# josh-holder/marl_sap

Measured on AMD Instinct MI355X. Metric: env steps/sec (whole node), 64-agent assignment env, 1/2/4/8 MI355X, higher is better.
Workload: dtype f32

## Files before the change

include/asg.h:

```cpp
#ifndef ASG_H
#define ASG_H

#include <stdint.h>

#ifdef __cplusplus
extern "C" {
#endif

#define ASG_ABI_VERSION 1

#define ASG_OK 0
#define ASG_E_INVALID_ARG (-1)
#define ASG_E_HIP (-2)
#define ASG_E_STATE (-3)
#define ASG_E_LSA_INVALID (-4)
#define ASG_E_LSA_INFEASIBLE (-5)
#define ASG_E_ACTION_RANGE (-6)

enum asg_dtype {
    ASG_F32 = 0,
    ASG_F64 = 1,
    ASG_I64 = 2,
    ASG_I32 = 3,
    ASG_BOOL = 4,
// ... 162 lines not shown
                          uint64_t seed, uint64_t counter, int64_t env_index_base, int64_t *out,
                          int32_t *status, void *hip_stream);

int asg_rollout(asg_handle *h, const asg_batch_view *b, int ts, int steps, int select_first, int select_last,
                const void *packed, const float *b1, const float *b_r0, const float *b_r1, const float *b2, int K,
                int hidden, int use_rnn, const float *h_in, int64_t h_stride, float *h_out, double epsilon,
                uint64_t seed, uint64_t counter, int32_t *status, void *hip_stream);
int asg_reset_rollout(asg_handle *h, const asg_batch_view *b, int ts, int steps, int select_last, const void *packed,
                      const float *b1, const float *b_r0, const float *b_r1, const float *b2, int K, int hidden,
                      int use_rnn, const float *h_in, int64_t h_stride, float *h_out, double epsilon, uint64_t seed,
                      uint64_t counter, int32_t *status, void *hip_stream);
int asg_step_select(asg_handle *h, const asg_batch_view *b, int ts, const void *packed, const float *b1,
                    const float *b_ih, const float *b_hh, const float *b2, int K, int hidden, const float *h_in,
                    int64_t h_stride, float *h_out, double epsilon, uint64_t seed, uint64_t counter,
                    int32_t *status, void *hip_stream);
int asg_step_forward(asg_handle *h, const asg_batch_view *b, int ts, const void *packed, const float *b1,
                     const float *b_r0, const float *b_r1, const float *b2, int K, int hidden, int use_rnn,
                     const float *h_in, int64_t h_stride, float *h_out, float *q_out, void *hip_stream);
int asg_step_forward_ex(asg_handle *h, const asg_batch_view *b, int ts, const void *packed, const float *b1,
                        const float *b_r0, const float *b_r1, const float *b2, int K, int hidden, int use_rnn,
                        const float *h_in, int64_t h_stride, float *h_out, float *q_out, int flags,
                        void *hip_stream);
int asg_reset_forward(asg_handle *h, const asg_batch_view *b, int ts, const void *packed, const float *b1,
                      const float *b_r0, const float *b_r1, const float *b2, int K, int hidden, int use_rnn,
                      const float *h_in, int64_t h_stride, float *h_out, float *q_out, void *hip_stream);
int asg_bids_select(asg_handle *h, const float *q, const int64_t q_strides[3], float *bids_out,
                    const int64_t out_strides[3], int row_softmax, int col_softmax, double noise_std, uint64_t seed,
                    uint64_t counter, void *hip_stream);
int asg_bids_select_count(asg_handle *h, const float *q, const int64_t q_strides[3], float *bids_out,
                          const int64_t out_strides[3], int row_softmax, int col_softmax, double noise_std,
                          uint64_t seed, uint64_t counter, int32_t *path_steps_out, void *hip_stream);
int asg_rollout_l2_slices(int n, int m, int L, int use_rnn);
int asg_step_select_l2_slices(int n, int m, int L);

typedef struct asg_real_handle asg_real_handle;

enum asg_real_variant { ASG_REAL_PLAIN = 0, ASG_REAL_POWER = 1, ASG_REAL_INTERFERENCE = 2 };

typedef struct {
    int64_t num_envs;
    int32_t n, m, T, L;
    int32_t N, M;
    double lambda_;
    const double *T_trans;
    const double *task_prios;
    int32_t variant;
    int32_t bids_as_actions;
    uint64_t seed;
    int64_t env_index_base;
    const int32_t *sat_freq_bands;
    const double *neighbor_matrix;
} asg_real_config;

typedef struct {
    asg_batch_view base;
    asg_field power_states;
} asg_real_batch_view;

int asg_real_create(const asg_real_config *cfg, int device, void *hip_stream, asg_real_handle **out);
void asg_real_destroy(asg_real_handle *h);
int asg_real_set_stream(asg_real_handle *h, void *hip_stream);
int asg_real_set_benefits(asg_real_handle *h, const double *table, int64_t count, int on_device);
int asg_real_set_initial_assignments(asg_real_handle *h, const int64_t *prev0, int64_t count, int on_device);
int asg_real_reset(asg_real_handle *h, const asg_real_batch_view *view, int ts);
int asg_real_step(asg_real_handle *h, const asg_real_batch_view *view, int ts);
int asg_real_sync_status(asg_real_handle *h);
// ... 12 lines not shown
```

marl_sap_amd/_lib.py:

```python
import ctypes
import os

import torch

HERE = os.path.dirname(os.path.abspath(__file__))
LIB_PATH = os.environ.get("ASG_LIB_PATH") or os.path.join(HERE, "libmarl_sap_amd.so")

ASG_OK = 0
ASG_E_INVALID_ARG = -1
ASG_E_HIP = -2
ASG_E_STATE = -3
ASG_E_LSA_INVALID = -4
ASG_E_LSA_INFEASIBLE = -5
ASG_E_ACTION_RANGE = -6

ASG_F32, ASG_F64, ASG_I64, ASG_I32, ASG_BOOL, ASG_F16, ASG_I16 = 0, 1, 2, 3, 4, 5, 6
ASG_RNG_PHILOX, ASG_RNG_MT19937 = 0, 1
ASG_BENEFIT_BUMP, ASG_BENEFIT_DENSE, ASG_BENEFIT_INJECTED = 0, 1, 2
ASG_QUIRK_PREV_ASSIGNS_ZERO = 0x1
ASG_QUIRK_PARALLEL_TERMINATED = 0x2
ASG_QUIRK_REPLICATE_STREAM = 0x4
ASG_STEP_USE_SELECTED_BIDS = 0x1

_DTYPES = {torch.float32: ASG_F32, torch.float64: ASG_F64, torch.int64: ASG_I64,
           torch.int32: ASG_I32, torch.bool: ASG_BOOL, torch.float16: ASG_F16, torch.int16: ASG_I16}

EXPORTS = ["asg_abi_version", "asg_last_error", "asg_create", "asg_destroy", "asg_set_stream",
           "asg_reset", "asg_step", "asg_random_actions", "asg_sync_status", "asg_set_benefits",
           "asg_export_benefits", "asg_export_bump_params", "asg_export_prev_assigns", "asg_get_returns", "asg_get_step",
           "asg_advance_stream", "asg_beta_hat", "asg_lsa_batched", "asg_haa_select", "asg_sap_select", "asg_epsilon_greedy",
           "asg_rnn_agent_packed_size", "asg_rnn_agent_mfma_mode", "asg_rnn_agent_mode", "asg_rnn_agent_pack", "asg_rnn_agent_forward",
           "asg_rnn_agent_select", "asg_real_create", "asg_real_destroy", "asg_real_set_stream",
           "asg_real_set_benefits", "asg_real_set_initial_assignments", "asg_real_reset", "asg_real_step", "asg_real_sync_status",
           "asg_real_get_returns", "asg_real_get_step", "asg_real_obs_size", "asg_filtered_topm",
           "asg_filtered_benefits", "asg_filtered_epsilon_greedy", "asg_filtered_soft_map", "asg_real_haal_select",
           "asg_real_haal_num_sequences", "asg_step_select", "asg_step_select_l2_slices", "asg_rollout",
           "asg_rollout_l2_slices", "asg_reset_rollout", "asg_sap_select_into", "asg_step_forward",
           "asg_sap_noise", "asg_random_rollout", "asg_sap_select_warm", "asg_bids_select",
           "asg_reset_forward", "asg_step_ex", "asg_step_forward_ex", "asg_bids_select_count",
           "asg_rnn_agent_unroll", "asg_rnn_agent_unroll_backward", "asg_mlp_agent_unroll",
           "asg_mlp_agent_unroll_backward", "asg_mlp_agent_unroll_ids", "asg_bids_log_prob", "asg_ppo_bids_loss",
           "asg_nstep_returns"]
ASG_PPO_ROWS_PER_GROUP = 16


class AsgField(ctypes.Structure):
    _fields_ = [("ptr", ctypes.c_void_p), ("dtype", ctypes.c_int32), ("pad_", ctypes.c_int32),
                ("stride", ctypes.c_int64 * 4)]


_VIEW_FIELDS = ["obs", "actions", "avail_actions", "rewards", "terminated", "prev_assigns", "beta",
                "actions_onehot", "filled"]


class AsgBatchView(ctypes.Structure):
    _fields_ = [(f, AsgField) for f in _VIEW_FIELDS]


class AsgConfig(ctypes.Structure):
    _fields_ = [("num_envs", ctypes.c_int64), ("n", ctypes.c_int32), ("m", ctypes.c_int32),
                ("T", ctypes.c_int32), ("L", ctypes.c_int32), ("lambda_", ctypes.c_double),
                ("bids_as_actions", ctypes.c_int32), ("rng_mode", ctypes.c_int32),
                ("benefit_mode", ctypes.c_int32), ("quirks", ctypes.c_uint32),
                ("seed", ctypes.c_uint64), ("env_index_base", ctypes.c_int64),
                ("T_trans", ctypes.POINTER(ctypes.c_double))]


class AsgRealConfig(ctypes.Structure):
    _fields_ = [("num_envs", ctypes.c_int64), ("n", ctypes.c_int32), ("m", ctypes.c_int32),
                ("T", ctypes.c_int32), ("L", ctypes.c_int32), ("N", ctypes.c_int32), ("M", ctypes.c_int32),
# ... 68 lines not shown
            L.asg_mlp_agent_unroll_backward.argtypes = [vp] * 4 + [i64, i32, vp, vp, vp]
        if hasattr(L, "asg_mlp_agent_unroll_ids"):
            L.asg_mlp_agent_unroll_ids.argtypes = L.asg_mlp_agent_unroll.argtypes
            L.asg_bids_log_prob.argtypes = [vp, vp, i64p, vp, i64p, i32, i64, i32, i32, dbl, i32, vp, vp]
            L.asg_ppo_bids_loss.argtypes = [vp, vp, i64p, vp, vp, vp, i64p, i32, i64, i32, i32, dbl, dbl, vp, i32, vp,
                                            vp, vp, vp]
            L.asg_nstep_returns.argtypes = [vp, vp, i64p, vp, i64p, i32, i64, i32, i32, dbl, i32, i32, vp, vp]
        L.asg_real_create.argtypes = [ctypes.POINTER(AsgRealConfig), i32, vp, ctypes.POINTER(vp)]
        L.asg_real_destroy.argtypes = [vp]
        L.asg_real_destroy.restype = None
        L.asg_real_set_stream.argtypes = [vp, vp]
        L.asg_real_set_benefits.argtypes = [vp, vp, i64, i32]
        L.asg_real_set_initial_assignments.argtypes = [vp, vp, i64, i32]
        L.asg_real_reset.argtypes = [vp, ctypes.POINTER(AsgRealBatchView), i32]
        L.asg_real_step.argtypes = [vp, ctypes.POINTER(AsgRealBatchView), i32]
        L.asg_real_sync_status.argtypes = [vp]
        L.asg_real_get_returns.argtypes = [vp, vp]
        L.asg_real_get_step.argtypes = [vp, ctypes.POINTER(ctypes.c_int)]
        L.asg_real_obs_size.argtypes = [i32, i32, i32]
        u64 = ctypes.c_uint64
        L.asg_filtered_topm.argtypes = [vp, i32, i64p, i64, i32, i32, i32, i32, vp, vp]
        L.asg_filtered_benefits.argtypes = [vp, i64p, vp, i64, i32, i32, i32, vp, dbl, vp, u64, u64, i64, vp, vp]
        L.asg_filtered_epsilon_greedy.argtypes = [vp, i64p, vp, i64p, i64, i32, i32, dbl, u64, u64, i64, vp, i64p,
                                                  vp, vp]
        L.asg_filtered_soft_map.argtypes = [vp, vp, i64, i32, i32, i32, u64, u64, i64, vp, vp, vp]
        L.asg_real_haal_select.argtypes = [vp, vp, vp, vp, vp]
        L.asg_real_haal_num_sequences.argtypes = [vp]
        L.asg_step_select.argtypes = [vp, ctypes.POINTER(AsgBatchView), i32, vp, vp, vp, vp, vp, i32, i32, vp, i64, vp,
                                      dbl, u64, u64, vp, vp]
        L.asg_step_select_l2_slices.argtypes = [i32, i32, i32]
        L.asg_rollout.argtypes = [vp, ctypes.POINTER(AsgBatchView), i32, i32, i32, i32, vp, vp, vp, vp, vp, i32, i32,
                                  i32, vp, i64, vp, dbl, u64, u64, vp, vp]
        L.asg_rollout_l2_slices.argtypes = [i32, i32, i32, i32]
        L.asg_reset_rollout.argtypes = [vp, ctypes.POINTER(AsgBatchView), i32, i32, i32, vp, vp, vp, vp, vp, i32, i32,
                                        i32, vp, i64, vp, dbl, u64, u64, vp, vp]
        L.asg_sap_select_into.argtypes = [vp, i64p, i64, i32, i32, dbl, u64, u64, i64, vp, vp, vp, vp]
        L.asg_sap_noise.argtypes = [vp, i64p, i64, i32, i32, dbl, u64, u64, i64, vp, vp, vp]
        if hasattr(L, "asg_sap_select_warm"):
            L.asg_sap_select_warm.argtypes = [vp, i64p, i64, i32, i32, dbl, u64, u64, i64, vp, vp, vp, vp, i32, vp]
        if hasattr(L, "asg_bids_select"):
            L.asg_bids_select.argtypes = [vp, vp, i64p, vp, i64p, i32, i32, dbl, u64, u64, vp]
        if hasattr(L, "asg_bids_select_count"):
            L.asg_bids_select_count.argtypes = [vp, vp, i64p, vp, i64p, i32, i32, dbl, u64, u64, vp, vp]
        if hasattr(L, "asg_reset_forward"):
            L.asg_reset_forward.argtypes = [vp, ctypes.POINTER(AsgBatchView), i32, vp, vp, vp, vp, vp, i32, i32, i32,
                                            vp, i64, vp, vp, vp]
        L.asg_step_forward.argtypes = [vp, ctypes.POINTER(AsgBatchView), i32, vp, vp, vp, vp, vp, i32, i32, i32, vp,
                                       i64, vp, vp, vp]
        if hasattr(L, "asg_step_ex"):
            L.asg_step_ex.argtypes = [vp, ctypes.POINTER(AsgBatchView), i32, i32]
            L.asg_step_forward_ex.argtypes = [vp, ctypes.POINTER(AsgBatchView), i32, vp, vp, vp, vp, vp, i32, i32,
                                              i32, vp, i64, vp, vp, i32, vp]
        for f in EXPORTS:
            if f not in ("asg_last_error", "asg_real_destroy") and hasattr(L, f):
                getattr(L, f).restype = i32
        L.asg_rnn_agent_packed_size.restype = i64
        if L.asg_abi_version() != 1:
            raise RuntimeError("libmarl_sap_amd.so ABI version mismatch")
        _lib = L
    return _lib


def last_error(handle=None):
    msg = lib().asg_last_error(handle)
    return msg.decode() if msg else ""

# ... 40 lines not shown
```

marl_sap_amd/csrc/asg_abi.hip:

```cpp
#include <hip/hip_runtime.h>

#include <cstdio>
#include <cstring>
#include <new>
#include <string>

#include "../../include/asg.h"
#include "asg_internal.h"

using asg::DeviceGuard;
using asg::EnvState;

struct asg_handle {
    EnvState st{};
    hipStream_t stream = nullptr;
    int device = 0;
    int k = 0;
    bool has_reset = false;
    bool constructed = false;
    bool table_ready = false;
    struct BidsTag {
        const float *row = nullptr;
        int64_t s_env = 0, s_agent = 0, s_task = 0;
    } bids_tag;
// ... 574 lines not shown
        return fail(nullptr, ASG_E_INVALID_ARG, "asg_filtered_epsilon_greedy: bad arguments");
    if (!(epsilon >= 0.0 && epsilon <= 1.0))
        return fail(nullptr, ASG_E_INVALID_ARG, "asg_filtered_epsilon_greedy: epsilon must be in [0, 1]");
    if (B == 0) return ASG_OK;
    hipError_t e = asg::launch_eps_greedy(mat, mat_strides, avail, avail_strides, B, n, m, (float)epsilon, seed,
                                          (uint32_t)counter, env_index_base * n, out, out_strides, status,
                                          static_cast<hipStream_t>(hip_stream), false);
    return e == hipSuccess ? ASG_OK : hip_fail(nullptr, e, "asg_filtered_epsilon_greedy");
}

int asg_filtered_soft_map(const int64_t *picked, const int64_t *topm, int64_t B, int n, int m, int M, uint64_t seed,
                          uint64_t counter, int64_t env_index_base, int64_t *out, int32_t *status, void *hip_stream) {
    if (!picked || !topm || !out || !status || B < 0 || n <= 0 || m <= 0 || env_index_base < 0)
        return fail(nullptr, ASG_E_INVALID_ARG, "asg_filtered_soft_map: bad arguments");
    if (M <= 0 || M >= m) return fail(nullptr, ASG_E_INVALID_ARG, "asg_filtered_soft_map: needs 1 <= M < m");
    if (B == 0) return ASG_OK;
    hipError_t e = asg::launch_filtered_soft_map(picked, topm, B, n, m, M, seed, (uint32_t)counter, env_index_base,
                                                 out, status, static_cast<hipStream_t>(hip_stream));
    return e == hipSuccess ? ASG_OK : hip_fail(nullptr, e, "asg_filtered_soft_map");
}

static void *tm_base(const asg_field &f, int64_t E, int64_t d2, int64_t d3, int64_t *row, bool *ok) {
    *row = 0;
    if (!f.ptr) return nullptr;
    const bool good = f.stride[0] == d2 * d3 && f.stride[1] == E * d2 * d3 && (d2 == 1 || f.stride[2] == d3) &&
                      (d3 == 1 || f.stride[3] == 1);
    if (!good) *ok = false;
    *row = f.stride[1];
    return f.ptr;
}

int asg_step_select_l2_slices(int n, int m, int L) { return asg::rollout_l2_slices(n, m, L, 1); }
int asg_rollout_l2_slices(int n, int m, int L, int use_rnn) { return asg::rollout_l2_slices(n, m, L, use_rnn); }

static int rollout_impl(asg_handle *h, const asg_batch_view *b, int ts, int steps, int select_first, int select_last,
                        int reset, const void *packed, const float *b1, const float *b_r0, const float *b_r1,
                        const float *b2, int K, int hidden, int use_rnn, const float *h_in, int64_t h_stride,
                        float *h_out, double epsilon, uint64_t seed, uint64_t counter, int32_t *status,
                        void *hip_stream, float *q_out = nullptr, int flags = 0) {
    if (!h) return fail(nullptr, ASG_E_INVALID_ARG, "NULL handle");
    if (int rc = check_view(h, b, ts, true)) return rc;
    if (flags & ~ASG_STEP_USE_SELECTED_BIDS) return fail(h, ASG_E_INVALID_ARG, "asg_step_forward_ex: unknown flags");
    if (reset && (flags & ASG_STEP_USE_SELECTED_BIDS))
        return fail(h, ASG_E_INVALID_ARG, "ASG_STEP_USE_SELECTED_BIDS: a reset has no bids row to step");
    if (int rc = selected_bids_ok(h, b, ts, flags)) return rc;
    if (!packed || !b1 || !b_r0 || (use_rnn && !b_r1) || !b2 || !h_out || (!status && !q_out))
        return fail(h, ASG_E_INVALID_ARG, "asg_rollout: NULL agent argument");
    if (q_out && (reinterpret_cast<uintptr_t>(q_out) % 16) != 0)
        return fail(h, ASG_E_INVALID_ARG, "asg_step_forward: q_out must be 16-B aligned");
    const asg::EnvState &st = h->st;
    if (!h->has_reset && !reset) return fail(h, ASG_E_STATE, "step called before reset");
    if (reset && st.rng_mode == ASG_RNG_PHILOX && st.benefit_mode == ASG_BENEFIT_INJECTED)
        return fail(h, ASG_E_INVALID_ARG, "asg_reset_rollout: not with an injected table in the Philox mode (asg_reset)");
    if (reset && st.benefit_mode == ASG_BENEFIT_INJECTED && !h->table_ready)
        return fail(h, ASG_E_STATE, "benefit_mode=injected needs asg_set_benefits before reset");
    const int k0 = reset ? 0 : h->k;
    const bool reset_forward = steps == 0 && reset && q_out;
    if ((steps < 1 && !reset_forward) || k0 + steps > st.T)
        return fail(h, ASG_E_STATE, "asg_rollout: steps must be >= 1 and stay within the episode (k + steps <= T)");
    if (select_first && k0 != 0)
        return fail(h, ASG_E_STATE, "asg_rollout: select_first selects on the reset row (k == 0 only)");
    if (select_last && k0 + steps >= st.T)
        return fail(h, ASG_E_STATE, "asg_rollout: select_last needs a next step to select for (k + steps < T)");
    if (ts < 0 || ts + steps > st.T)
        return fail(h, ASG_E_INVALID_ARG, "asg_rollout: batch rows ts .. ts + steps must lie in the [T + 1]-row batch");
    if (st.bids && !q_out)
// ... 132 lines not shown
```

marl_sap_amd/csrc/asg_h2.hip:

```cpp
#include "rollout_tile.h"

#pragma clang fp contract(fast)

namespace asg {

H2Geom h2_geom(int K, int nout) {
    H2Geom g;
    g.K = K;
    g.nout = nout;
    g.nct = (nout + 15) / 16;
    const bool blocked = nout >= 16 && K % nout == 0 && K / nout >= 2;
    g.P = blocked ? nout : K;
    g.NB = blocked ? K / nout : 1;
    g.prefix = blocked ? 1 : 0;
    g.Pp = (g.P + 31) / 32 * 32;
    g.Kp = g.Pp * g.NB;
    return g;
}
bool h2_ok(int K, int nout) { return K >= 1 && nout >= 1 && nout <= 256; }
int64_t h2_packed_f4(int K, int nout, int use_rnn) {
    const H2Geom g = h2_geom(K, nout);
    return w1t_f4(g) + 1 + w1s_f4(g.Kp) + rec_f4(use_rnn != 0) + w2s_f4(g.nct);
}

// ... 115 lines not shown
    const int64_t ntiles = (R + kH2Waves * 16 * kH2NT - 1) / (kH2Waves * 16 * kH2NT);
    const unsigned grid = (unsigned)(ntiles < ncu ? ntiles : ncu);
    if (grid == 0) return hipSuccess;
#define LH_(RNN, SEL, W2L, GEN) \
    hipLaunchKernelGGL((rnn_agent_h2_kernel<RNN, SEL, W2L, GEN>), dim3(grid), dim3(64 * kH2Waves), plan.bytes, s, ha)
#define LH2_(RNN, SEL)                                                      \
    do {                                                                    \
        if (plan.w2l) {                                                     \
            if (gen) LH_(RNN, SEL, true, true); else LH_(RNN, SEL, true, false);   \
        } else {                                                            \
            if (gen) LH_(RNN, SEL, false, true); else LH_(RNN, SEL, false, false); \
        }                                                                   \
    } while (0)
    if (rnn) {
        if (sel) LH2_(true, true); else LH2_(true, false);
    } else {
        if (sel) LH2_(false, true); else LH2_(false, false);
    }
#undef LH2_
#undef LH_
    return hipGetLastError();
}

bool rollout_shape_ok(int n, int m, int L, int K) {
    if (n < 1 || m < 16 || m > 256 || n > 256 || L < 1 || K != m * (L + 1) || !h2_ok(K, m)) return false;
    return onehot_prefix_enabled() && h2_geom(K, m).prefix;
}

int rollout_l2_slices(int n, int m, int L, int use_rnn) {
    if (!rollout_shape_ok(n, m, L, m * (L + 1))) return -1;
    const H2Geom g = h2_geom(m * (L + 1), m);
    const int64_t scr = ((int64_t)rollout_scratch_bytes(n, m) * kH2Waves + 15) / 16;
    return h2_lds_plan(g, use_rnn != 0, g.Pp / 32, scr).l2_slices;
}

hipError_t launch_rollout(const RolloutSlabs &sl, const EnvState &st, int ts, int k0, int steps, int select_first,
                          int select_last, int reset, const float4 *packed, const float *b1, const float *bi, const float *bh,
                          const float *b2, int use_rnn, const float *Hin, int64_t hs, float *Hout, float *Q, float epsilon,
                          uint64_t seed, uint32_t counter, int64_t row_base, int *err, hipStream_t s) {
    const int K = st.m * (st.L + 1), nout = st.m;
    const H2Geom g = h2_geom(K, nout);
    const bool rnn = use_rnn != 0;
    RolloutArgs ra{};
    ra.obs = sl.obs;
    ra.beta = sl.beta;
    ra.avail = sl.avail;
    ra.onehot = sl.onehot;
    ra.act = sl.act;
    ra.rew = sl.rew;
    ra.prevb = sl.prevb;
    ra.term = sl.term;
    ra.filled = sl.filled;
    ra.ts0 = ts;
    ra.prev = st.prev;
    ra.returns = st.returns;
    ra.T_trans = st.T_trans;
    ra.env_err = st.err;
    ra.lambda_ = st.lambda_;
    ra.seed = st.seed;
    ra.env_base = st.env_base;
    ra.E = st.E;
    ra.episode = st.episode;
    ra.quirks = st.quirks;
    ra.n = st.n;
    ra.m = st.m;
    ra.T = st.T;
// ... 22 lines not shown
    ra.W1T = reinterpret_cast<const float *>(packed);
    ra.pk = reinterpret_cast<const u32x4v *>(packed + w1t_f4(g));
    ra.Hin = Hin;
    ra.hs = hs;
    ra.Hout = Hout;
    ra.b1 = b1;
    ra.bi = bi;
    ra.bh = bh;
    ra.b2 = b2;
    ra.epsilon = epsilon;
    ra.sk0 = (uint32_t)seed;
    ra.sk1 = (uint32_t)(seed >> 32) ^ 0x5bd1e995u;
    ra.counter = counter;
    (void)row_base;
    ra.sel_err = err;
    const int64_t scr_f4 = ((int64_t)rollout_scratch_bytes(st.n, st.m) * kH2Waves + 15) / 16;
    const H2Lds plan = h2_lds_plan(g, rnn, g.Pp / 32, scr_f4);
    ra.w1_lds = plan.w1_lds;
    ra.w1_off = 0;
    ra.scratch_off = plan.scratch_off;
    const int ncu = stream_cus(s);
    RolloutLaunch lc;
    lc.lds = plan.bytes;
    lc.rnn = rnn;
    lc.w2l = plan.w2l;
    lc.gen = st.m % 32 != 0 || st.n % 32 != 0;
    lc.sq64 = st.n == 64 && st.m == 64 && plan.w2l;
    int passes = 0;
    for (int it = 0, nit = steps + (select_first ? 1 : 0); it < nit; ++it) {
        const int kk = k0 + it - (select_first ? 1 : 0) + 1;
        passes += kk < st.T && (kk < ra.k1 || select_last);
    }
    lc.pair = lc.sq64 && !Q && passes >= 2;
    const int per_wg = lc.pair ? kH2Waves / 2 : kH2Waves;
    const int64_t wgs = (st.E + per_wg - 1) / per_wg;
    lc.grid = (unsigned)(wgs < ncu ? wgs : ncu);
    if (lc.sq64 && plan.l2_slices >= 1) ra.w1_off = 1;
    if (Q) return launch_rollout_q(ra, lc, s);
    if (tab) return launch_rollout_tab(ra, lc, s);
    return launch_rollout_inst<0, false>(ra, lc, s);
}

}
```

marl_sap_amd/csrc/asg_internal.h:

```cpp
#pragma once
#include <hip/hip_runtime.h>
#include <stdint.h>

#include <string>

#include "../../include/asg.h"

namespace asg {

void set_last_error(const std::string &msg);

struct DeviceGuard {
    int prev = -1;
    explicit DeviceGuard(int dev) {
        if (hipGetDevice(&prev) != hipSuccess) prev = -1;
        if (prev != dev) (void)hipSetDevice(dev);
    }
    ~DeviceGuard() {
        int cur = -1;
        if (prev >= 0 && hipGetDevice(&cur) == hipSuccess && cur != prev) (void)hipSetDevice(prev);
    }
};

struct EnvState {
// ... 94 lines not shown
    int K, P, NB, Pp, Kp, prefix, nout, nct;
};
H2Geom h2_geom(int K, int nout);
bool h2_ok(int K, int nout);
int64_t h2_packed_f4(int K, int nout, int use_rnn);
hipError_t launch_h2_pack(const float *W1, const float *Wih, const float *Whh, const float *W2, int K, int nout,
                          int use_rnn, float4 *packed, hipStream_t s);
hipError_t launch_h2_agent(const float *X, int64_t xs, int64_t R, int K, const float *Hin, int64_t hs,
                           const float4 *packed, const float *b1, const float *bih, const float *bhh, const float *b2,
                           int nout, int use_rnn, float *Hout, float *Q, const SelectArgs *sel, hipStream_t s);

struct RolloutSlabs {
    float *obs;
    int64_t obs_row;
    float *beta;
    int64_t beta_row;
    uint8_t *avail;
    int64_t avail_row;
    int64_t *onehot;
    int64_t onehot_row;
    int64_t *act;
    int64_t act_row;
    float *rew;
    int64_t rew_row;
    int64_t *prevb;
    int64_t prevb_row;
    uint8_t *term;
    int64_t term_row;
    int64_t *filled;
    int64_t filled_row;
};
bool rollout_shape_ok(int n, int m, int L, int K);
int rollout_l2_slices(int n, int m, int L, int use_rnn);
hipError_t launch_rollout(const RolloutSlabs &sl, const EnvState &st, int ts, int k0, int steps, int select_first,
                          int select_last, int reset, const float4 *packed, const float *b1, const float *bi, const float *bh,
                          const float *b2, int use_rnn, const float *Hin, int64_t hs, float *Hout, float *Q,
                          float epsilon, uint64_t seed, uint32_t counter, int64_t row_base, int *err, hipStream_t s);
hipError_t launch_rnn_agent_pack(const float *W1, const float *Wih, const float *Whh, const float *W2, int K, int nout,
                                 int use_rnn, float4 *packed, hipStream_t s);
hipError_t launch_rnn_agent_fwd(const float *X, int64_t xs, int64_t R, int K, const float *Hin, int64_t hs,
                                const float4 *packed, const float *b1, const float *bih, const float *bhh,
                                const float *b2, int nout, int use_rnn, float *Hout, float *Q,
                                const SelectArgs *sel, hipStream_t s);
hipError_t launch_rnn_agent_select(const float *X, int64_t xs, int64_t R, int K, const float *Hin, int64_t hs,
                                   const float4 *packed, const float *b1, const float *bih, const float *bhh,
                                   const float *b2, int nout, int use_rnn, float *Hout, float *Q,
                                   const uint8_t *avail, int64_t a0, int64_t a1, int n, float epsilon, uint64_t seed,
                                   uint32_t counter, int64_t row_base, int64_t *out, int64_t o0, int64_t o1, int *err,
                                   hipStream_t s);

}
```

marl_sap_amd/csrc/h2_tile.h:

```cpp
#pragma once
#include <type_traits>

#include "asg_agent_common.h"

#pragma clang fp contract(fast)

namespace asg {

typedef _Float16 f16x8 __attribute__((ext_vector_type(8)));
typedef _Float16 f16x2v __attribute__((ext_vector_type(2)));
typedef long long i64x2v __attribute__((ext_vector_type(2)));
typedef const u32x4v __attribute__((address_space(3))) * lds_u4p;
typedef const f32x4 __attribute__((address_space(3))) * lds_f4v;

__device__ __forceinline__ f32x4 mfma_h(const u32x4v &a, const u32x4v &b, f32x4 c) {
    return __builtin_amdgcn_mfma_f32_16x16x32_f16(__builtin_bit_cast(f16x8, a), __builtin_bit_cast(f16x8, b), c, 0, 0,
                                                  0);
}
__device__ __forceinline__ f32x4 mfma_h2(const u32x4v (&w)[2], const u32x4v (&x)[2], f32x4 c) {
    c = mfma_h(w[1], x[0], c);
    c = mfma_h(w[0], x[1], c);
    c = mfma_h(w[0], x[0], c);
    return c;
}
// ... 629 lines not shown
            }
        }
        if (attempt == 0 && RNN) load_h();
        bool over[NT], any = false;
#pragma unroll
        for (int nt = 0; nt < NT; ++nt) {
            const float rm = row_max4(rmax[nt]);
            over[nt] = rm * scx[nt] >= 32768.f;
            any = any || over[nt];
            if (over[nt]) sx[nt] = h2_scale(rm, -90, 90 - sw[0]);
        }
        if (attempt > 0 || __ballot(any) == 0) break;
    }
    f32x4 xB[4][NT];
#pragma unroll
    for (int nt = 0; nt < NT; ++nt) {
        const float un = pow2f(-(sw[0] + sx[nt]));
#pragma unroll
        for (int mt = 0; mt < 4; ++mt) {
            const f32x4 bb = Bs[4 * mt + q];
#pragma unroll
            for (int v = 0; v < 4; ++v) xB[mt][nt][v] = fmaxf(acc[mt][nt][v] * un + bb[v], 0.f);
        }
    }
    h2_tail<NT, RNN, SEL, W2L, false, GEN>(a, Wl, sw, row0, rows, ok, hB, xB);
}

struct H2Lds {
    bool w2l;
    int w1_lds, l2_slices;
    int64_t scratch_off;
    size_t bytes;
};
static inline H2Lds h2_lds_plan(const H2Geom &g, bool rnn, int s0, int64_t reserve_f4) {
    constexpr int64_t kCap = 160 * 1024 / 16;
    H2Lds p{};
    p.w2l = lds_w2_off(rnn, g.nct) + w2s_f4(g.nct) + reserve_f4 <= kCap;
    const int64_t w1off = lds_w1_off(rnn, g.nct, p.w2l);
    const int64_t slices = g.Kp / 32 - s0, fit = (kCap - reserve_f4 - w1off) / (4 * 2 * 64);
    p.w1_lds = (int)(fit < slices ? (fit > 0 ? fit : 0) : slices);
    p.l2_slices = (int)(slices - p.w1_lds);
    p.scratch_off = w1off + (int64_t)p.w1_lds * 4 * 2 * 64;
    p.bytes = (size_t)(p.scratch_off + reserve_f4) * 16;
    return p;
}

}
```

marl_sap_amd/csrc/rollout_tile.h:

```cpp
#pragma once
#include "h2_tile.h"

#pragma clang fp contract(fast)

namespace asg {

struct RolloutArgs {
    float *obs, *beta, *rew;
    uint8_t *avail, *term;
    int64_t *onehot, *act, *prevb, *filled;
    int ts0;
    int *prev;
    double *returns;
    const double *T_trans;
    int *env_err;
    double lambda_;
    uint64_t seed;
    int64_t env_base, E;
    uint32_t episode, quirks;
    int n, m, T, L, dense;
    float wmin, wmax;
    int k0, k1, select_first, select_last;
    int reset;
    const double *table;
    const double2 *par;
    const float *table32;
    const uint64_t *tmask;
    const int *toff;
    float *Q;
    const u32x4v *pk;
    const float *W1T, *Hin;
    int64_t hs;
    float *Hout;
    const float *b1, *bi, *bh, *b2;
    int w1_lds, w1_off;
    float epsilon;
    uint32_t sk0, sk1, counter;
    int *sel_err;
    int64_t scratch_off;
    const int *assign;
};

typedef __attribute__((address_space(4))) const RolloutArgs KRolloutArgs;
__device__ __forceinline__ KRolloutArgs &rollout_args(KRolloutArgs *p) {
    asm volatile("" : "+s"(p));
    return *p;
}

__host__ __device__ constexpr int rollout_mp(int m) { return (m + 31) / 32 * 32; }
__host__ __device__ constexpr int rollout_np(int n) { return (n + 31) / 32 * 32; }
__host__ __device__ constexpr int rollout_scratch_bytes(int n, int m) {
    return (40 + 4 * rollout_mp(m) + 4 * rollout_np(n) + 15) / 16 * 16;
}

__device__ __forceinline__ void wave_lds_fence() {
    __builtin_amdgcn_fence(__ATOMIC_RELEASE, "wavefront");
    __builtin_amdgcn_wave_barrier();
    __builtin_amdgcn_fence(__ATOMIC_ACQUIRE, "wavefront");
}

template <int SQ, class RA>
__device__ __forceinline__ int rs_n(RA &ra) { return SQ ? SQ : ra.n; }
template <int SQ, class RA>
__device__ __forceinline__ int rs_m(RA &ra) { return SQ ? SQ : ra.m; }

template <int SQ = 0, class RA>
__device__ __forceinline__ H2Args rollout_h2args(RA &ra) {
    H2Args a{};
    const int n = rs_n<SQ>(ra), m = rs_m<SQ>(ra), L = ra.L;
    a.R = ra.E * n;
    a.g.K = m * (L + 1);
    a.g.P = m;
// ... 7 lines not shown
    a.pk = ra.pk;
    a.W1T = ra.W1T;
    a.b1 = ra.b1;
    a.bi = ra.bi;
    a.bh = ra.bh;
    a.b2 = ra.b2;
    a.Hout = ra.Hout;
    a.w1_lds = ra.w1_lds;
    a.w1_off = ra.w1_off;
    a.sel = SelectArgs{nullptr, 0, 0, n, ra.epsilon, ra.sk0, ra.sk1, ra.counter, ra.env_base * n, nullptr,
                       (int64_t)n, 1, ra.sel_err};
    return a;
}

__device__ __forceinline__ float task_scale(const uint64_t *s_scl, int j) {
    return ((s_scl[j >> 6] >> (j & 63)) & 1ull) ? 10.0f : 1.0f;
}

template <class RA>
__device__ __forceinline__ void rollout_actions_from_batch(RA &ra, int64_t e, int ts, uint16_t *s_act) {
    const int lane = threadIdx.x & 63;
    const int n = ra.n, m = ra.m;
    int err = 0;
    for (int i = lane; i < n; i += 64) {
        const int64_t a64 = ra.assign ? (int64_t)ra.assign[e * n + i] : ra.act[((int64_t)ts * ra.E + e) * n + i];
        int a = (a64 >= 0 && a64 < m) ? (int)a64 : -1;
        if (a < 0) err = ASG_E_ACTION_RANGE;
        s_act[i] = (uint16_t)(a < 0 ? 0 : a);
    }
    err = wave_or_i32(err);
    if (lane == 0 && err) atomicCAS(ra.env_err, 0, err);
}

template <int TAB, int SQ, class RA>
__device__ __forceinline__ void rollout_transition(RA &ra, int64_t e, int k, int ts, const EnvKey &key,
                                                   const uint64_t *s_scl, int *s_cnt, uint16_t *s_act,
                                                   uint16_t *s_prev, double *s_ret) {
    asm volatile("" : "+s"(e), "+s"(ts));
    int lane_ = threadIdx.x & 63;
    asm volatile("" : "+v"(lane_));
    const int lane = lane_;
    const int n = rs_n<SQ>(ra), m = rs_m<SQ>(ra), mp = rollout_mp(m);
    for (int j = lane; j < mp; j += 64) s_cnt[j] = 0;
    wave_lds_fence();
    for (int i = lane; i < n; i += 64) atomicAdd(&s_cnt[s_act[i]], 1);
    wave_lds_fence();
    const BumpShape bsh = bump_shape(ra.T, ra.wmin, ra.wmax);
    (void)bsh;
    double sum = 0.0;
    auto rewards = [&](auto with_table) {
        constexpr bool TT = decltype(with_table)::value;
        for (int i0 = 0; i0 < n; i0 += 64) {
            const int i = i0 + lane;
            double rr = 0.0;
            if (i < n) {
                const int j = s_act[i], p = s_prev[i];
                double beta;
                if constexpr (TAB) {
                    beta = ra.par ? mt_par_value(ra.par[(e * m + j) * n + i], k)
                                  : ra.table[(((int64_t)e * ra.T + k) * n + i) * m + j];
                } else if (ASG_ROLLOUT_XSKIP & 1024) {
                    beta = (double)(j & 3) * 0.25;
                } else {
                    const Bump32 b =
                        philox_bump32(key, ra.episode, i * m + j, task_scale(s_scl, j), bsh, ra.dense != 0);
                    beta = bump64_at(b, k);
                }
                const double tt = TT ? ra.T_trans[(int64_t)p * m + j] : (j == p ? 0.0 : 1.0);
                const double pen = tt * (beta > 1e-12 ? 1.0 : 0.0);
                const double bh = beta - ra.lambda_ * pen;
                rr = bh > 0.0 ? bh / (double)s_cnt[j] : bh;
                if (ra.rew) ra.rew[((int64_t)ts * ra.E + e) * n + i] = (float)rr;
                s_prev[i] = (uint16_t)j;
                if (ra.prevb)
                    ra.prevb[((int64_t)(ts + 1) * ra.E + e) * n + i] =
                        (ra.quirks & ASG_QUIRK_PREV_ASSIGNS_ZERO) ? 0 : j;
            }
            const int lo = __double2loint(rr), hi = __double2hiint(rr);
            const int cnt = n - i0 < 64 ? n - i0 : 64;
            for (int l2 = 0; l2 < ((ASG_ROLLOUT_XSKIP & 512) ? 1 : cnt); ++l2)
                sum += __hiloint2double(__builtin_amdgcn_readlane(hi, l2), __builtin_amdgcn_readlane(lo, l2));
        }
    };
    if (ra.T_trans) rewards(std::true_type{});
    else rewards(std::false_type{});
    if (lane == 0) {
        *s_ret += sum;
        bool term = k + 1 >= ra.T;
        if (ra.quirks & ASG_QUIRK_PARALLEL_TERMINATED) term = (e != 0);
        if (ra.term) ra.term[(int64_t)ts * ra.E + e] = term;
        if (ra.filled) ra.filled[(int64_t)(ts + 1) * ra.E + e] = 1;
    }
    wave_lds_fence();
}

__device__ __forceinline__ void st_f4(float *p, float a, float b, float c, float d) {
    *reinterpret_cast<f32x4 *>(p) = f32x4{a, b, c, d};
}
__device__ __forceinline__ void st_i64x2(int64_t *p, long long a, long long b) {
    *reinterpret_cast<i64x2v *>(p) = i64x2v{a, b};
}

__device__ __forceinline__ void tile_action_rows64(float *ob, int64_t *oh, uint8_t *av, int K, const uint16_t *sa,
                                                   bool have_act) {
    constexpr int RT = 16 * kH2NT, M = 64;
    int lane = threadIdx.x & 63;
    asm volatile("" : "+v"(lane));
    {
        const int rl = lane >> 4, c0 = 4 * (lane & 15);
        const uint32_t lo = (uint32_t)(rl * K + c0);
        const int cc = have_act ? c0 : 0x10000;
#pragma unroll
        for (int i = 0; i < RT / 4; ++i) {
            const int d = (int)sa[4 * i + rl] - cc;
            st_f4(ob + (uint32_t)(4 * i * K) + lo, d == 0, d == 1, d == 2, d == 3);
        }
    }
    if (oh) {
        const int rl = lane >> 5, c0 = 2 * (lane & 31);
        const uint32_t lo = (uint32_t)(2 * lane);
// ... 513 lines not shown
                for (int sub = 0; sub < ntile; ++sub) {
                    HNext nx{nullptr, kHid, 0, 0};
                    if (sub + 1 < ntile) nx = HNext{pass == 0 ? ri.Hin : ri.Hout, pass == 0 ? ri.hs : kHid,
                                                    (int64_t)(16 * kH2NT) * (sub + 1), 1};
                    else if (next_agent) nx = HNext{ri.Hout, kHid, 0, 1};
                    rollout_tile<RNN, W2L, GEN, TAB, QOUT, true, SQ>(rollout_args(kra), e, sub, kk, ts + 1,
                                                                     !first_sel || ri.reset, !first_sel, pass, key, s_scl,
                                                                     s_act, s_act, s_h2, sw, hN, hpf, nx);
                    hpf = nx.mode != 0;
                }
                ++pass;
            } else {
                for (int sub = 0; sub < ntile; ++sub)
                    rollout_tile<RNN, W2L, GEN, TAB, QOUT, false, SQ>(rollout_args(kra), e, sub, kk, ts + 1, true, true, 0,
                                                                      key, s_scl, s_act, s_act, s_h2, sw, hN, false,
                                                                      HNext{nullptr, kHid, 0, 0});
            }
            wave_lds_fence();
        }
        for (int i = lane; i < n; i += 64) ra.prev[e * n + i] = s_prev[i];
        if (lane == 0) ra.returns[e] = *s_ret;
        wave_lds_fence();
    }
}

__device__ __forceinline__ void pair_barrier() {
    __builtin_amdgcn_fence(__ATOMIC_RELEASE, "wavefront");
    asm volatile("s_waitcnt lgkmcnt(0)" ::: "memory");
    __builtin_amdgcn_s_barrier();
    asm volatile("" ::: "memory");
    __builtin_amdgcn_fence(__ATOMIC_ACQUIRE, "wavefront");
}

constexpr int kPairScratchBytes = 720;
static_assert(kPairScratchBytes <= 2 * rollout_scratch_bytes(64, 64), "pair scratch: two wave slots");

template <bool RNN, bool W2L, int TAB, bool QOUT>
__device__ __forceinline__ void rollout_envs_pair(const RolloutArgs &ra, u32x4v *s_h2, const int (&sw)[4]) {
    constexpr int SQ = 64, n = 64, m = 64;
    const int lane = threadIdx.x & 63, wv = __builtin_amdgcn_readfirstlane(threadIdx.x >> 6);
    const int pr = wv >> 1, sub = wv & 1;
    const bool trw = sub == (pr >> 1);
    char *scr = reinterpret_cast<char *>(s_h2 + ra.scratch_off) + pr * (2 * rollout_scratch_bytes(n, m));
    uint64_t *s_scl = reinterpret_cast<uint64_t *>(scr + 32 * sub);
    double *s_ret = reinterpret_cast<double *>(scr + 64);
    int *s_cnt = reinterpret_cast<int *>(scr + 80);
    uint16_t *s_act2 = reinterpret_cast<uint16_t *>(scr + 336);
    uint16_t *s_prev = reinterpret_cast<uint16_t *>(scr + 592);
    constexpr int kPairs = kH2Waves / 2;
    const int64_t GP = (int64_t)gridDim.x * kPairs;
    for (int64_t eb = (int64_t)blockIdx.x * kPairs; eb < ra.E; eb += GP) {
        int64_t e = eb + pr;
        asm volatile("" : "+s"(e));
        const bool active = e < ra.E;
        const EnvKey key = env_key(ra.seed, ra.env_base + e);
        if (active) {
            if (!TAB) {
                const bool ten = philox_task_scale(key, ra.episode, lane) == 10.0f;
                const uint64_t bits = __ballot(ten);
                if (lane == 0) s_scl[0] = bits;
            }
            if (trw) {
                if (!TAB && ra.reset) {
                    uint16_t *s_perm = reinterpret_cast<uint16_t *>(s_cnt), *s_jj = s_perm + m;
                    s_perm[lane] = (uint16_t)lane;
                    const u32x4 rr = philox4x32_10(u32x4{(uint32_t)lane, 0u, kCtrPerm, ra.episode}, key.k0, key.k1);
                    s_jj[lane] = (uint16_t)(((uint64_t)rr.x * (uint64_t)(lane + 1)) >> 32);
                    wave_lds_fence();
                    if (lane == 0)
                        for (int i = m - 1; i >= 1; --i) {
                            const int jj = s_jj[i];
                            const uint16_t t = s_perm[i];
                            s_perm[i] = s_perm[jj];
                            s_perm[jj] = t;
                        }
                    wave_lds_fence();
                    const int p = (int)s_perm[lane];
                    s_prev[lane] = (uint16_t)p;
                    if (ra.prevb)
                        ra.prevb[((int64_t)ra.ts0 * ra.E + e) * n + lane] = (ra.quirks & ASG_QUIRK_PREV_ASSIGNS_ZERO) ? 0 : p;
                    if (lane == 0 && ra.filled) ra.filled[(int64_t)ra.ts0 * ra.E + e] = 1;
                } else {
                    const int p = ra.prev[e * n + lane];
                    s_prev[lane] = (uint16_t)p;
                    if (TAB && ra.reset && ra.prevb)
                        ra.prevb[((int64_t)ra.ts0 * ra.E + e) * n + lane] = (ra.quirks & ASG_QUIRK_PREV_ASSIGNS_ZERO) ? 0 : p;
                    if (TAB && ra.reset && lane == 0 && ra.filled) ra.filled[(int64_t)ra.ts0 * ra.E + e] = 1;
                }
                s_act2[lane] = 0;
                if (lane == 0) *s_ret = ra.reset ? 0.0 : ra.returns[e];
                if (!ra.select_first) rollout_actions_from_batch(ra, e, ra.ts0, s_act2);
            }
        }
        wave_lds_fence();
        pair_barrier();
        KRolloutArgs *const kra = (KRolloutArgs *)__builtin_amdgcn_kernarg_segment_ptr();
        const int sf = ra.select_first ? 1 : 0;
        const int nit = ra.k1 - ra.k0 + sf;
        int pass = 0;
        f32x4 hN[4][kH2NT];
        auto has_agent = [&](auto &rr, int it) {
            const int kk = rr.k0 + it - sf + 1;
            return it < nit && kk < rr.T && (kk < rr.k1 || rr.select_last);
        };
        for (int it = 0; it < nit; ++it) {
            auto &ri = rollout_args(kra);
            const int k = ri.k0 + it - sf;
            const int ts = ri.ts0 + (k - ri.k0);
            const bool first_sel = it < sf;
            const bool agent = has_agent(ri, it);
            uint16_t *const sa = s_act2 + n * (pass & 1), *const saw = s_act2 + n * ((pass & 1) ^ 1);
            if (active) {
                if (trw && !first_sel && !(ASG_ROLLOUT_XSKIP & 256))
                    rollout_transition<TAB, SQ>(rollout_args(kra), e, k, ts, key, s_scl, s_cnt, sa, s_prev, s_ret);
                const int kk = k + 1;
                if (agent) {
                    const int last = __builtin_amdgcn_readfirstlane(has_agent(ri, it + 1) ? 0 : 1);
                    rollout_tile<RNN, W2L, false, TAB, QOUT, true, SQ>(rollout_args(kra), e, sub, kk, ts + 1,
                                                                       !first_sel || ri.reset, !first_sel, pass, key, s_scl,
                                                                       sa, saw, s_h2, sw, hN, pass > 0,
                                                                       HKeep{last});
                } else {
                    rollout_tile<RNN, W2L, false, TAB, QOUT, false, SQ>(rollout_args(kra), e, sub, kk, ts + 1, true, true, 0,
                                                                        key, s_scl, sa, saw, s_h2, sw, hN, false,
                                                                        HKeep{0});
                }
            }
            if (agent) ++pass;
            wave_lds_fence();
            pair_barrier();
        }
        if (active && trw) {
            ra.prev[e * n + lane] = s_prev[lane];
            if (lane == 0) ra.returns[e] = *s_ret;
        }
        wave_lds_fence();
    }
}

template <bool RNN, bool W2L, bool GEN, int TAB, bool QOUT, int SQ, bool PAIR = false>
__global__ void __launch_bounds__(64 * kH2Waves) __attribute__((amdgpu_waves_per_eu(kH2WavesPerSimd)))
rollout_kernel(RolloutArgs ra) {
    static_assert(!PAIR || (SQ == 64 && !GEN && !QOUT), "the wave-pair mapping: n = m = 64, selecting instances");
    extern __shared__ u32x4v s_h2[];
    int sw[4];
    h2_stage<RNN, W2L>(rollout_h2args(ra), s_h2, sw);
    __syncthreads();
    if constexpr (PAIR) rollout_envs_pair<RNN, W2L, TAB, QOUT>(ra, s_h2, sw);
    else rollout_envs_wave<RNN, W2L, GEN, TAB, QOUT, SQ>(ra, s_h2, sw);
}

struct RolloutLaunch {
    unsigned grid;
    size_t lds;
    bool rnn, w2l, gen;
    bool sq64;
    bool pair;
};
template <int TAB, bool QOUT>
static hipError_t launch_rollout_inst(const RolloutArgs &ra, const RolloutLaunch &lc, hipStream_t s) {
#define LR_(RNN, W2L, GEN, SQ, PAIR)                                                                            \
    hipLaunchKernelGGL((rollout_kernel<RNN, W2L, GEN, TAB, QOUT, SQ, PAIR>), dim3(lc.grid), dim3(64 * kH2Waves), lc.lds, \
                       s, ra)
#define LR2_(RNN)                                                                              \
    do {                                                                                       \
        if (lc.sq64 && lc.pair) {                                                              \
            if constexpr (QOUT) return hipErrorInvalidValue;    \
            else LR_(RNN, true, false, 64, true);                                              \
        } else if (lc.sq64) {                                                                  \
// ... 17 lines not shown
```

Baseline: 34.62 million.

## Defer env transitions in paired rollout to batch them across steps

In the wave-pair rollout path, the per-step environment transition (reward, previous-assignment update) is taken out of the agent loop. Actions for up to G steps are recorded in an LDS history buffer, and the transitions for that group are then computed in one pass, split across the two waves of the pair by alternating steps. This is meant to cut the number of pair barriers, and the serialized transition work on one wave, from once per step to a couple per group. In exchange it needs more LDS scratch, sized from the remaining capacity, which may grow the LDS allocation, and it makes the bookkeeping for returns and the previous assignment more intricate.

Measured after the change: 35.15 million (median of 6 runs). +1.5%, better.

```diff
diff --git a/include/asg.h b/include/asg.h
--- a/include/asg.h
+++ b/include/asg.h
@@ -218,6 +218,7 @@
                           uint64_t seed, uint64_t counter, int32_t *path_steps_out, void *hip_stream);
 int asg_rollout_l2_slices(int n, int m, int L, int use_rnn);
 int asg_step_select_l2_slices(int n, int m, int L);
+int asg_rollout_defer_steps(int n, int m, int L, int use_rnn);
 
 typedef struct asg_real_handle asg_real_handle;
 
diff --git a/marl_sap_amd/_lib.py b/marl_sap_amd/_lib.py
--- a/marl_sap_amd/_lib.py
+++ b/marl_sap_amd/_lib.py
@@ -35,7 +35,7 @@
            "asg_real_get_returns", "asg_real_get_step", "asg_real_obs_size", "asg_filtered_topm",
            "asg_filtered_benefits", "asg_filtered_epsilon_greedy", "asg_filtered_soft_map", "asg_real_haal_select",
            "asg_real_haal_num_sequences", "asg_step_select", "asg_step_select_l2_slices", "asg_rollout",
-           "asg_rollout_l2_slices", "asg_reset_rollout", "asg_sap_select_into", "asg_step_forward",
+           "asg_rollout_l2_slices", "asg_rollout_defer_steps", "asg_reset_rollout", "asg_sap_select_into", "asg_step_forward",
            "asg_sap_noise", "asg_random_rollout", "asg_sap_select_warm", "asg_bids_select",
            "asg_reset_forward", "asg_step_ex", "asg_step_forward_ex", "asg_bids_select_count",
            "asg_rnn_agent_unroll", "asg_rnn_agent_unroll_backward", "asg_mlp_agent_unroll",
@@ -170,6 +170,8 @@
         L.asg_rollout.argtypes = [vp, ctypes.POINTER(AsgBatchView), i32, i32, i32, i32, vp, vp, vp, vp, vp, i32, i32,
                                   i32, vp, i64, vp, dbl, u64, u64, vp, vp]
         L.asg_rollout_l2_slices.argtypes = [i32, i32, i32, i32]
+        if hasattr(L, "asg_rollout_defer_steps"):
+            L.asg_rollout_defer_steps.argtypes = [i32, i32, i32, i32]
         L.asg_reset_rollout.argtypes = [vp, ctypes.POINTER(AsgBatchView), i32, i32, i32, vp, vp, vp, vp, vp, i32, i32,
                                         i32, vp, i64, vp, dbl, u64, u64, vp, vp]
         L.asg_sap_select_into.argtypes = [vp, i64p, i64, i32, i32, dbl, u64, u64, i64, vp, vp, vp, vp]
diff --git a/marl_sap_amd/csrc/asg_abi.hip b/marl_sap_amd/csrc/asg_abi.hip
--- a/marl_sap_amd/csrc/asg_abi.hip
+++ b/marl_sap_amd/csrc/asg_abi.hip
@@ -630,6 +630,7 @@
 
 int asg_step_select_l2_slices(int n, int m, int L) { return asg::rollout_l2_slices(n, m, L, 1); }
 int asg_rollout_l2_slices(int n, int m, int L, int use_rnn) { return asg::rollout_l2_slices(n, m, L, use_rnn); }
+int asg_rollout_defer_steps(int n, int m, int L, int use_rnn) { return asg::rollout_defer_steps(n, m, L, use_rnn); }
 
 static int rollout_impl(asg_handle *h, const asg_batch_view *b, int ts, int steps, int select_first, int select_last,
                         int reset, const void *packed, const float *b1, const float *b_r0, const float *b_r1,
diff --git a/marl_sap_amd/csrc/asg_h2.hip b/marl_sap_amd/csrc/asg_h2.hip
--- a/marl_sap_amd/csrc/asg_h2.hip
+++ b/marl_sap_amd/csrc/asg_h2.hip
@@ -171,6 +171,18 @@
     const H2Geom g = h2_geom(m * (L + 1), m);
     const int64_t scr = ((int64_t)rollout_scratch_bytes(n, m) * kH2Waves + 15) / 16;
     return h2_lds_plan(g, use_rnn != 0, g.Pp / 32, scr).l2_slices;
+}
+
+int rollout_defer_steps(int n, int m, int L, int use_rnn) {
+    if (n != 64 || m != 64 || !rollout_shape_ok(n, m, L, m * (L + 1))) return 0;
+    const H2Geom g = h2_geom(m * (L + 1), m);
+    const int64_t scr = ((int64_t)rollout_scratch_bytes(n, m) * kH2Waves + 15) / 16;
+    const H2Lds plan = h2_lds_plan(g, use_rnn != 0, g.Pp / 32, scr);
+    if (!plan.w2l) return 0;
+    const int64_t room = (kH2LdsBytes - plan.scratch_off * 16) / (kH2Waves / 2);
+    int G = kMaxDeferSteps;
+    while (G > 0 && pair_scratch_bytes(G) > room) --G;
+    return G;
 }
 
 hipError_t launch_rollout(const RolloutSlabs &sl, const EnvState &st, int ts, int k0, int steps, int select_first,
@@ -259,6 +271,12 @@
         passes += kk < st.T && (kk < ra.k1 || select_last);
     }
     lc.pair = lc.sq64 && !Q && passes >= 2;
+    if (lc.pair) {
+        ra.defer = rollout_defer_steps(st.n, st.m, st.L, use_rnn);
+        if (ra.defer < 1) return hipErrorInvalidValue;
+        const int64_t pair_f4 = (int64_t)pair_scratch_bytes(ra.defer) * (kH2Waves / 2) / 16;
+        if (pair_f4 > scr_f4) lc.lds = (size_t)(plan.scratch_off + pair_f4) * 16;
+    }
     const int per_wg = lc.pair ? kH2Waves / 2 : kH2Waves;
     const int64_t wgs = (st.E + per_wg - 1) / per_wg;
     lc.grid = (unsigned)(wgs < ncu ? wgs : ncu);
diff --git a/marl_sap_amd/csrc/asg_internal.h b/marl_sap_amd/csrc/asg_internal.h
--- a/marl_sap_amd/csrc/asg_internal.h
+++ b/marl_sap_amd/csrc/asg_internal.h
@@ -150,6 +150,7 @@
 };
 bool rollout_shape_ok(int n, int m, int L, int K);
 int rollout_l2_slices(int n, int m, int L, int use_rnn);
+int rollout_defer_steps(int n, int m, int L, int use_rnn);
 hipError_t launch_rollout(const RolloutSlabs &sl, const EnvState &st, int ts, int k0, int steps, int select_first,
                           int select_last, int reset, const float4 *packed, const float *b1, const float *bi, const float *bh,
                           const float *b2, int use_rnn, const float *Hin, int64_t hs, float *Hout, float *Q,
diff --git a/marl_sap_amd/csrc/h2_tile.h b/marl_sap_amd/csrc/h2_tile.h
--- a/marl_sap_amd/csrc/h2_tile.h
+++ b/marl_sap_amd/csrc/h2_tile.h
@@ -685,8 +685,9 @@
     int64_t scratch_off;
     size_t bytes;
 };
+constexpr int64_t kH2LdsBytes = 160 * 1024;
 static inline H2Lds h2_lds_plan(const H2Geom &g, bool rnn, int s0, int64_t reserve_f4) {
-    constexpr int64_t kCap = 160 * 1024 / 16;
+    constexpr int64_t kCap = kH2LdsBytes / 16;
     H2Lds p{};
     p.w2l = lds_w2_off(rnn, g.nct) + w2s_f4(g.nct) + reserve_f4 <= kCap;
     const int64_t w1off = lds_w1_off(rnn, g.nct, p.w2l);
diff --git a/marl_sap_amd/csrc/rollout_tile.h b/marl_sap_amd/csrc/rollout_tile.h
--- a/marl_sap_amd/csrc/rollout_tile.h
+++ b/marl_sap_amd/csrc/rollout_tile.h
@@ -38,6 +38,7 @@
     uint32_t sk0, sk1, counter;
     int *sel_err;
     int64_t scratch_off;
+    int defer;
     const int *assign;
 };
 
@@ -111,7 +112,7 @@
     if (lane == 0 && err) atomicCAS(ra.env_err, 0, err);
 }
 
-template <int TAB, int SQ, class RA>
+template <int TAB, int SQ, bool DEFER = false, class RA>
 __device__ __forceinline__ void rollout_transition(RA &ra, int64_t e, int k, int ts, const EnvKey &key,
                                                    const uint64_t *s_scl, int *s_cnt, uint16_t *s_act,
                                                    uint16_t *s_prev, double *s_ret) {
@@ -150,7 +151,7 @@
                 const double bh = beta - ra.lambda_ * pen;
                 rr = bh > 0.0 ? bh / (double)s_cnt[j] : bh;
                 if (ra.rew) ra.rew[((int64_t)ts * ra.E + e) * n + i] = (float)rr;
-                s_prev[i] = (uint16_t)j;
+                if (!DEFER) s_prev[i] = (uint16_t)j;
                 if (ra.prevb)
                     ra.prevb[((int64_t)(ts + 1) * ra.E + e) * n + i] =
                         (ra.quirks & ASG_QUIRK_PREV_ASSIGNS_ZERO) ? 0 : j;
@@ -164,7 +165,8 @@
     if (ra.T_trans) rewards(std::true_type{});
     else rewards(std::false_type{});
     if (lane == 0) {
-        *s_ret += sum;
+        if (DEFER) *s_ret = sum;
+        else *s_ret += sum;
         bool term = k + 1 >= ra.T;
         if (ra.quirks & ASG_QUIRK_PARALLEL_TERMINATED) term = (e != 0);
         if (ra.term) ra.term[(int64_t)ts * ra.E + e] = term;
@@ -744,21 +746,26 @@
     __builtin_amdgcn_fence(__ATOMIC_ACQUIRE, "wavefront");
 }
 
-constexpr int kPairScratchBytes = 720;
-static_assert(kPairScratchBytes <= 2 * rollout_scratch_bytes(64, 64), "pair scratch: two wave slots");
+constexpr int kPairHistOff = 672;
+constexpr int kPairRow = 68;
+constexpr int kMaxDeferSteps = 16;
+__host__ __device__ constexpr int pair_scratch_bytes(int G) {
+    return (kPairHistOff + 2 * kPairRow * G + 128 + 15) / 16 * 16;
+}
 
 template <bool RNN, bool W2L, int TAB, bool QOUT>
 __device__ __forceinline__ void rollout_envs_pair(const RolloutArgs &ra, u32x4v *s_h2, const int (&sw)[4]) {
     constexpr int SQ = 64, n = 64, m = 64;
-    const int lane = threadIdx.x & 63, wv = __builtin_amdgcn_readfirstlane(threadIdx.x >> 6);
+    const int wv = __builtin_amdgcn_readfirstlane(threadIdx.x >> 6);
     const int pr = wv >> 1, sub = wv & 1;
     const bool trw = sub == (pr >> 1);
-    char *scr = reinterpret_cast<char *>(s_h2 + ra.scratch_off) + pr * (2 * rollout_scratch_bytes(n, m));
-    uint64_t *s_scl = reinterpret_cast<uint64_t *>(scr + 32 * sub);
-    double *s_ret = reinterpret_cast<double *>(scr + 64);
-    int *s_cnt = reinterpret_cast<int *>(scr + 80);
-    uint16_t *s_act2 = reinterpret_cast<uint16_t *>(scr + 336);
-    uint16_t *s_prev = reinterpret_cast<uint16_t *>(scr + 592);
+    char *scr = reinterpret_cast<char *>(s_h2 + ra.scratch_off) + pr * pair_scratch_bytes(ra.defer);
+    uint64_t *s_scl = reinterpret_cast<uint64_t *>(scr + 8 * sub);
+    double *s_ret = reinterpret_cast<double *>(scr + 16);
+    int *s_cnt = reinterpret_cast<int *>(scr + 32 + 256 * sub);
+    uint16_t *s_prev = reinterpret_cast<uint16_t *>(scr + 544);
+    uint16_t *s_hist = reinterpret_cast<uint16_t *>(scr + kPairHistOff);
+    auto s_sum = [&](int j) { return reinterpret_cast<double *>(s_hist + kPairRow * j + 64); };
     constexpr int kPairs = kH2Waves / 2;
     const int64_t GP = (int64_t)gridDim.x * kPairs;
     for (int64_t eb = (int64_t)blockIdx.x * kPairs; eb < ra.E; eb += GP) {
@@ -766,6 +773,8 @@
         asm volatile("" : "+s"(e));
         const bool active = e < ra.E;
         const EnvKey key = env_key(ra.seed, ra.env_base + e);
+        int lane = threadIdx.x & 63;
+        asm volatile("" : "+v"(lane));
         if (active) {
             if (!TAB) {
                 const bool ten = philox_task_scale(key, ra.episode, lane) == 10.0f;
@@ -799,9 +808,9 @@
                         ra.prevb[((int64_t)ra.ts0 * ra.E + e) * n + lane] = (ra.quirks & ASG_QUIRK_PREV_ASSIGNS_ZERO) ? 0 : p;
                     if (TAB && ra.reset && lane == 0 && ra.filled) ra.filled[(int64_t)ra.ts0 * ra.E + e] = 1;
                 }
-                s_act2[lane] = 0;
+                s_hist[lane] = 0;
                 if (lane == 0) *s_ret = ra.reset ? 0.0 : ra.returns[e];
-                if (!ra.select_first) rollout_actions_from_batch(ra, e, ra.ts0, s_act2);
+                if (!ra.select_first) rollout_actions_from_batch(ra, e, ra.ts0, s_hist);
             }
         }
         wave_lds_fence();
@@ -809,44 +818,78 @@
         KRolloutArgs *const kra = (KRolloutArgs *)__builtin_amdgcn_kernarg_segment_ptr();
         const int sf = ra.select_first ? 1 : 0;
         const int nit = ra.k1 - ra.k0 + sf;
-        int pass = 0;
         f32x4 hN[4][kH2NT];
         auto has_agent = [&](auto &rr, int it) {
             const int kk = rr.k0 + it - sf + 1;
             return it < nit && kk < rr.T && (kk < rr.k1 || rr.select_last);
         };
-        for (int it = 0; it < nit; ++it) {
-            auto &ri = rollout_args(kra);
-            const int k = ri.k0 + it - sf;
-            const int ts = ri.ts0 + (k - ri.k0);
-            const bool first_sel = it < sf;
-            const bool agent = has_agent(ri, it);
-            uint16_t *const sa = s_act2 + n * (pass & 1), *const saw = s_act2 + n * ((pass & 1) ^ 1);
+        for (int g0 = 0; g0 < nit; g0 += rollout_args(kra).defer) {
+            const int gn = min(rollout_args(kra).defer, nit - g0);
+            for (int j = 0; j < gn; ++j) {
+                const int it = g0 + j, pass = it;
+                auto &ri = rollout_args(kra);
+                const int k = ri.k0 + it - sf;
+                const int ts = ri.ts0 + (k - ri.k0);
+                const bool first_sel = it < sf;
+                const bool agent = has_agent(ri, it);
+                uint16_t *const sa = s_hist + kPairRow * j, *const saw = sa + kPairRow;
+                if (active) {
+                    const int kk = k + 1;
+                    if (agent) {
+                        const int last = __builtin_amdgcn_readfirstlane(has_agent(ri, it + 1) ? 0 : 1);
+                        rollout_tile<RNN, W2L, false, TAB, QOUT, true, SQ>(rollout_args(kra), e, sub, kk, ts + 1,
+                                                                           !first_sel || ri.reset, !first_sel, pass, key,
+                                                                           s_scl, sa, saw, s_h2, sw, hN, pass > 0,
+                                                                           HKeep{last});
+                    } else {
+                        rollout_tile<RNN, W2L, false, TAB, QOUT, false, SQ>(rollout_args(kra), e, sub, kk, ts + 1, true, true,
+                                                                            0, key, s_scl, sa, saw, s_h2, sw, hN, false,
+                                                                            HKeep{0});
+                    }
+                }
+                wave_lds_fence();
+            }
+            pair_barrier();
+            int lane = threadIdx.x & 63;
+            asm volatile("" : "+v"(lane));
+            const int own = 32 * sub + (lane & 31);
+            const bool moved = g0 + gn > sf;
+            uint16_t t_last = 0, t_next = 0;
             if (active) {
-                if (trw && !first_sel && !(ASG_ROLLOUT_XSKIP & 256))
-                    rollout_transition<TAB, SQ>(rollout_args(kra), e, k, ts, key, s_scl, s_cnt, sa, s_prev, s_ret);
-                const int kk = k + 1;
-                if (agent) {
-                    const int last = __builtin_amdgcn_readfirstlane(has_agent(ri, it + 1) ? 0 : 1);
-                    rollout_tile<RNN, W2L, false, TAB, QOUT, true, SQ>(rollout_args(kra), e, sub, kk, ts + 1,
-                                                                       !first_sel || ri.reset, !first_sel, pass, key, s_scl,
-                                                                       sa, saw, s_h2, sw, hN, pass > 0,
-                                                                       HKeep{last});
-                } else {
-                    rollout_tile<RNN, W2L, false, TAB, QOUT, false, SQ>(rollout_args(kra), e, sub, kk, ts + 1, true, true, 0,
-                                                                        key, s_scl, sa, saw, s_h2, sw, hN, false,
-                                                                        HKeep{0});
-                }
-            }
-            if (agent) ++pass;
+                for (int j = (sub + g0) & 1; j < gn; j += 2) {
+                    const int it = g0 + j;
+                    if (it < sf || (ASG_ROLLOUT_XSKIP & 256)) continue;
+                    auto &ri = rollout_args(kra);
+                    const int k = ri.k0 + it - sf;
+                    const int ts = ri.ts0 + (k - ri.k0);
+                    uint16_t *const pv = (j == 0 || it - 1 < sf) ? s_prev : s_hist + kPairRow * (j - 1);
+                    rollout_transition<TAB, SQ, true>(rollout_args(kra), e, k, ts, key, s_scl, s_cnt, s_hist + kPairRow * j,
+                                                      pv, s_sum(j));
+                }
+                t_last = moved ? s_hist[kPairRow * (gn - 1) + own] : s_prev[own];
+                t_next = s_hist[kPairRow * gn + own];
+            }
+            pair_barrier();
+            if (active) {
+                const bool more = g0 + gn < nit;
+                if (lane < 32) {
+                    if (more) {
+                        s_prev[own] = t_last;
+                        s_hist[own] = t_next;
+                    } else {
+                        ra.prev[e * n + own] = t_last;
+                    }
+                }
+                if (trw && lane == 0) {
+                    double ret = *s_ret;
+                    for (int j = 0; j < gn; ++j)
+                        if (g0 + j >= sf && !(ASG_ROLLOUT_XSKIP & 256)) ret += *s_sum(j);
+                    *s_ret = ret;
+                    if (!more) ra.returns[e] = ret;
+                }
+            }
             wave_lds_fence();
-            pair_barrier();
-        }
-        if (active && trw) {
-            ra.prev[e * n + lane] = s_prev[lane];
-            if (lane == 0) ra.returns[e] = *s_ret;
-        }
-        wave_lds_fence();
+        }
     }
 }
 
```
